# otaviog/align3d

Measured on AMD Instinct MI355X. Metric: ICP frame-pairs/sec (640x480, 3-lvl, 15 iters), higher is better.
Workload: dtype f32; 1 GPU; ms3x15 x 64 pairs/GPU, distinct frames, 640x480, 3 lvl x 15 it, HBM-resident (configs[4] shard); pairs_per_gpu=64, global_pairs=64, levels=3, distinct_frames=True, ranks_in_collective=1, collective=none

## Files before the change

align3d_amd/csrc/image_icp.hip:

```cpp
#include <cstdlib>
#include <memory>

#include "icp_engine.hpp"

using namespace a3d;

namespace {

struct LevelDesc {
  const float* src_points;
  const uint8_t* src_mask;
  const uint8_t* src_intensities;
  const float* tgt_points;
  const float* tgt_normals;
  const uint8_t* tgt_mask;
  const float* imap;
  uint32_t src_n;
  uint32_t tw, th;
  float fx, fy, cx, cy;
  uint32_t flags;
  uint32_t ppt;
  uint32_t src_w;
  const uint16_t* src_depth;
  const uint16_t* tgt_depth;
// ... 61 lines not shown
  uint32_t depth;
  float row, col;
};
struct SrcStride {
  float q, q1, r, w;
};
__device__ __forceinline__ SrcStride make_src_stride(uint32_t w) {
  w = w ? w : 1u;
  const uint32_t q = 256u / w;
  return {(float)q, (float)(q + 1u), (float)(256u - q * w), (float)w};
}
__device__ __forceinline__ void src_advance(const SrcStride& st, float row, float col, float* nrow, float* ncol) {
  const float c = col + st.r;
  const bool wrap = c >= st.w;
  *ncol = wrap ? c - st.w : c;
  *nrow = row + (wrap ? st.q1 : st.q);
}
struct BackProj {
  float fx, fy, cx, cy, scale;
  DivBy dfx, dfy;
};
struct BackProj2 {
  BackProj src, tgt;
};
__device__ __forceinline__ float uniform_f(float x) {
  return __int_as_float(__builtin_amdgcn_readfirstlane(__float_as_int(x)));
}
template <bool SHORT = false>
__device__ __forceinline__ BackProj make_backproj(const float (&k)[5], const float (&rcp_f)[2]) {
  BackProj b;
  b.fx = k[0], b.fy = k[1], b.cx = k[2], b.cy = k[3], b.scale = k[4];
  if (SHORT) {
    b.dfx = DivBy{-b.fx, rcp_f[0]}, b.dfy = DivBy{-b.fy, rcp_f[1]};
    return b;
  }
  const DivBy dx = div_prepare(b.fx), dy = div_prepare(b.fy);
  b.dfx = DivBy{uniform_f(dx.negz), uniform_f(dx.y)}, b.dfy = DivBy{uniform_f(dy.negz), uniform_f(dy.y)};
  return b;
}
constexpr int D16_TGT = 1, D16_SRC = 2;
#ifndef A3D_ICP_DEPTH16_SRC
#define A3D_ICP_DEPTH16_SRC 1
#endif
constexpr int D16_SIDES = D16_TGT | (A3D_ICP_DEPTH16_SRC ? D16_SRC : 0);
template <bool ZMASK = false, int D16 = 0>
__device__ __forceinline__ SrcPx stage_a(const LevelDesc& d, uint32_t i, bool in_range, const SrcPx* prev = nullptr,
                                         const SrcStride* stride = nullptr) {
  const uint32_t ii = in_range ? i : 0u;
  SrcPx s;
  if (D16 & D16_SRC) {
    if (prev) {
      src_advance(*stride, prev->row, prev->col, &s.row, &s.col);
    } else {
      const uint32_t r = f32_as_usize(((float)i + 0.5f) * d.src_inv_w);
      s.row = (float)r, s.col = (float)(i - __umul24(r, d.src_w));
    }
    s.depth = ld<uint16_t>(d.src_depth, ii * 2u);
    s.intensity = ld<uint8_t>(d.src_intensities, ii);
    s.live = in_range;
    return s;
  }
  s.sp = ld_v3(d.src_points, ii);
  s.intensity = ld<uint8_t>(d.src_intensities, ii);
  if (ZMASK) {
    s.live = in_range & (s.sp.z != 0.0f);
    return s;
  }
  const uint8_t mask = ld<uint8_t>(d.src_mask, ii);
  s.live = in_range & (mask != 0);
  return s;
}

struct ProjPx {
  V3 p;
  float u, v;
  V3 tp, tn;
  uint8_t tmask;
  bool live;
  _Float16 tdepth;
  uint32_t trow, tcol;
  float t00, t10, t01, t11;
};
template <bool ZMASK = false, int D16 = 0, bool CLASSIC = false, bool SHORT = false>
__device__ __forceinline__ ProjPx stage_b(const LevelDesc& d, const Pose& T, const SrcPx& s, float twf, float thf,
                                          const BackProj2& bp = BackProj2{}) {
  ProjPx o;
  V3 sp = s.sp;
  bool slive = s.live;
  if (D16 & D16_SRC) {
    sp = backproject_px_proven_f<SHORT>((float)s.depth, s.row, s.col, bp.src.cx, bp.src.cy, bp.src.scale, bp.src.dfx, bp.src.dfy);
    slive = slive & (s.depth != 0u);
  }
  o.p = transform_vector(T, sp);
  const float z = o.p.z, au = o.p.x * d.fx, av = o.p.y * d.fy;
  const DivBy dz = div_prepare(z);
  float qu = div_by(au, dz), qv = div_by(av, dz);
  if (__builtin_expect(__builtin_amdgcn_ballot_w64(!(div_den_ok(z) & div_num_ok(au) & div_num_ok(av))) != 0ull, 0))
    qu = au / z, qv = av / z;
  o.u = qu + d.cx;
  o.v = qv + d.cy;
  const float ur = o.u + 0.5f, vr = o.v + 0.5f;
  o.live = slive & !((ur <= -1.0f) | (ur >= twf) | (vr <= -1.0f) | (vr >= thf));
  const uint32_t col = (uint32_t)f32_as_i32(ur), row = (uint32_t)f32_as_i32(vr);
  const uint32_t tidx = o.live ? __umul24(row, d.tw) + col : 0u;
  if (D16 & D16_TGT) {
    o.tdepth = ld<_Float16>(d.tgt_depth, tidx * 2u);
    o.trow = row, o.tcol = col;
    o.tn = ld_v3(d.tgt_normals, tidx);
// ... 234 lines not shown
  if (st->status != A3D_OK) sa.mode = SOLVE_NONE;
  block_finish<NACC>(acc, partials + (size_t)pair * gridDim.x * GN_PARTIAL, tile, gridDim.x,
                     counters + pair, st, sa, pair);
}

__global__ void __launch_bounds__(256)
    image_icp_exact_kernel(const LevelDesc* __restrict__ descs, const JobState* __restrict__ states, Gates gt,
                           float* __restrict__ partials, int PPT) {
  float acc[GN_PARTIAL];
#pragma unroll
  for (int k = 0; k < GN_PARTIAL; ++k) acc[k] = 0.0f;
  const LevelDesc d = descs[0];
  const Pose T = states[0].pose;
  const uint32_t mw = d.tw + 2;
  const float twf = (float)d.tw, thf = (float)d.th;
  auto step_exact = [](float* a, float r, const float J[6]) {
    int t = 0;
    for (int i = 0; i < 6; ++i)
      for (int j = i; j < 6; ++j) {
        const float m = J[i] * J[j];
        a[t] = a[t] + m;
        ++t;
      }
    for (int i = 0; i < 6; ++i) {
      const float m = J[i] * r;
      a[21 + i] = a[21 + i] + m;
    }
    const float rr = r * r;
    a[27] = a[27] + rr;
    a[28] += 1.0f;
  };
  for (int k0 = 0; k0 < PPT; ++k0) {
    const uint32_t i = blockIdx.x * (256u * (uint32_t)PPT) + threadIdx.x + (uint32_t)k0 * 256u;
    const SrcPx s0 = stage_a(d, i, i < d.src_n);
    ProjPx px = stage_b(d, T, s0, twf, thf);
    const MapPx mp = stage_c(d, gt, px, mw);
    if (px.live) {
      const Terms t = stage_d<true>(d, gt, px, mp, s0.intensity, mw);
      step_exact(acc, t.rg, t.Jg);
      if (t.color) step_exact(acc + GN_ACC, t.rc, t.Jc);
    }
  }
  block_reduce_store<GN_PARTIAL, false>(acc, partials + (size_t)blockIdx.x * GN_PARTIAL);
}

#endif

template <bool ZMASK, int D16 = 0>
__device__ __forceinline__ SrcPx pixel_source_at(const LevelDesc& d, uint32_t base, int ppt, int k0,
                                                 const SrcPx* prev = nullptr, const SrcStride* stride = nullptr) {
  const uint32_t i = base + (uint32_t)k0 * 256u;
  return stage_a<ZMASK, D16>(d, i, (k0 < ppt) && (i < d.src_n), prev, stride);
}
template <bool ZMASK, int D16 = 0, bool CLASSIC = false, bool SHORT = false, bool LATE = false>
__device__ __forceinline__ void pixel_pass(const LevelDesc& d, const Gates& gt, const Pose& T, uint32_t base, int ppt,
                                           const SrcPx& s0, SrcPx sa, float (&acc)[GN_PARTIAL]) {
  const uint32_t mw = d.tw + 2;
  const float twf = (float)d.tw, thf = (float)d.th;
  BackProj2 bp{};
  if (D16 & D16_SRC) bp.src = make_backproj<SHORT>(d.src_bp, d.src_rcp_f);
  if (D16 & D16_TGT) bp.tgt = make_backproj<SHORT>(d.tgt_bp, d.tgt_rcp_f);
  SrcStride stride{};
  if (D16 & D16_SRC) stride = make_src_stride(d.src_w);
  SrcPx sb;
  ProjPx pa = stage_b<ZMASK, D16, CLASSIC, SHORT>(d, T, s0, twf, thf, bp), pb;
  uint8_t ia = s0.intensity, ib;
  auto step = [&](ProjPx& cur, uint8_t cur_i, ProjPx& nxt, uint8_t& nxt_i, const SrcPx& s_next, SrcPx& s_new, int k0) {
    Shifted sh;
    if constexpr (!CLASSIC && !LATE) sh = request_shifted(d, cur, mw);
    s_new = pixel_source_at<ZMASK, D16>(d, base, ppt, k0 + 2, &s_next, &stride);
    if constexpr (!CLASSIC) {
      __builtin_amdgcn_sched_barrier(0);
      nxt = stage_b<ZMASK, D16, false, SHORT>(d, T, s_next, twf, thf, bp);
      nxt_i = s_next.intensity;
      __builtin_amdgcn_sched_barrier(0);
      const MapPx mp = stage_c<ZMASK, D16, false, SHORT>(d, gt, cur, mw, bp, LATE ? nullptr : &sh);
      if (cur.live) {
        const Terms t = stage_d(d, gt, cur, mp, cur_i, mw, LATE ? nullptr : &sh);
        gn_step(acc, t.rg, t.Jg);
        if (t.color) gn_step(acc + GN_ACC, t.rc, t.Jc);
      }
      return;
    }
    if (D16) __builtin_amdgcn_sched_barrier(0);
    const MapPx mp = stage_c<ZMASK, D16, true, SHORT>(d, gt, cur, mw, bp);
    nxt = stage_b<ZMASK, D16, true, SHORT>(d, T, s_next, twf, thf, bp);
    nxt_i = s_next.intensity;
    if (cur.live) {
      const Terms t = stage_d(d, gt, cur, mp, cur_i, mw);
      gn_step(acc, t.rg, t.Jg);
      if (t.color) gn_step(acc + GN_ACC, t.rc, t.Jc);
    }
  };
#pragma unroll 1
  for (int k0 = 0; k0 < ppt; k0 += 2) {
    step(pa, ia, pb, ib, sa, sb, k0);
    step(pb, ib, pa, ia, sb, sa, k0 + 1);
  }
}

template <bool ZMASK, bool DEPTH16, bool CLASSIC = false, bool SHORT = false, bool LATE = false>
__global__ void __launch_bounds__(256, 1)
    image_icp_head_kernel(const LevelDesc* __restrict__ descs, const JobState* __restrict__ states_in,
                          JobState* __restrict__ states_out, Gates gt, const float* __restrict__ partials_in,
                          float* __restrict__ partials_out, uint32_t job_stride, HeadArgs head) {
  __shared__ uint32_t s_state[JOB_WORDS];
  const int pair = blockIdx.y;
  const uint32_t tile = blockIdx.x;
  float acc[GN_PARTIAL];
#pragma unroll
  for (int k = 0; k < GN_PARTIAL; ++k) acc[k] = 0.0f;
#if defined(A3D_DIAGNOSTICS) && defined(A3D_TAIL_STAMPS)
  const bool stamping = threadIdx.x == 0 && pair == 0 && tile + 1 == gridDim.x;
  unsigned long long* stamp = g_tail_stamps + 16 + 8 * ((states_out > states_in) ? 1 : 0);
#define A3D_HEAD_STAMP(k) do { if (stamping) stamp[k] = __builtin_amdgcn_s_memrealtime(); } while (0)
#else
#define A3D_HEAD_STAMP(k) do { } while (0)
#endif
  A3D_HEAD_STAMP(0);
  const LevelDesc d = descs[pair];
  const int ppt = (int)d.ppt;
  const uint32_t base = tile * (256u * (uint32_t)ppt) + threadIdx.x;
  constexpr int D16 = DEPTH16 ? D16_SIDES : 0;
  SrcStride stride{};
  if (D16 & D16_SRC) stride = make_src_stride(d.src_w);
  const SrcPx s0 = pixel_source_at<ZMASK, D16>(d, base, ppt, 0), s1 = pixel_source_at<ZMASK, D16>(d, base, ppt, 1, &s0, &stride);
  A3D_HEAD_STAMP(1);
  head_advance(states_in + pair, tile == 0 ? states_out + pair : nullptr, partials_in + (size_t)pair * job_stride, head,
               pair, s_state, tile == 0);
  A3D_HEAD_STAMP(2);
  if ((int)s_state[15] == A3D_OK) {
    auto uni = [&](int k) { return __uint_as_float(__builtin_amdgcn_readfirstlane(s_state[k])); };
    const Pose T{{uni(0), uni(1), uni(2)}, {uni(3), uni(4), uni(5), uni(6)}};
    pixel_pass<ZMASK, D16, CLASSIC, SHORT, LATE>(d, gt, T, base, ppt, s0, s1, acc);
  }
  A3D_HEAD_STAMP(3);
  block_reduce_store<GN_PARTIAL, false>(acc, partials_out + (size_t)pair * job_stride + (size_t)tile * GN_PARTIAL);
  A3D_HEAD_STAMP(4);
#undef A3D_HEAD_STAMP
}

#ifdef A3D_DIAGNOSTICS
struct PersistLevel {
  uint32_t desc_base;
  uint32_t iterations;
  uint32_t tiles;
  float weight, color_weight;
  Gates gates;
};
constexpr int PERSIST_MAX_LEVELS = 16;
constexpr uint32_t PAIR_CTRL_WORDS = 64;
constexpr uint32_t ROSTER_CLOSED = 0x80000000u;
constexpr unsigned long long ROSTER_WAIT_TICKS = 2000ull, PERSIST_SPIN_BOUND_TICKS = 200'000'000ull;
struct PersistPlan {
  uint32_t n_levels;
  uint32_t seq0;
  uint32_t counter_base;
  uint32_t finish;
  uint32_t parity;
  int trace_index0;
  int trace_stride;
  HeadArgs prev;
  PersistLevel lv[PERSIST_MAX_LEVELS];
};
struct PersistOut {
  Pose* poses;
  int32_t* status;
  float* matrices;
  unsigned long long* stamps;
};

template <bool ZMASK>
__global__ void __launch_bounds__(256, 4)
    image_icp_persistent_kernel(const LevelDesc* __restrict__ descs, uint32_t n_pairs_total, JobState* __restrict__ states,
                                float* __restrict__ partials, uint32_t partials_half, uint32_t job_stride,
                                unsigned* __restrict__ ctrl, PersistPlan plan, PersistOut out) {
  __shared__ uint32_t s_state[JOB_WORDS];
  __shared__ uint32_t s_rank, s_members;
  __shared__ int s_go;
  const int pair = blockIdx.y;
  unsigned* const counter = ctrl + (size_t)pair * PAIR_CTRL_WORDS;
  unsigned* const roster = counter + 1 + plan.parity;
  unsigned* const members = counter + 3 + plan.parity;
  float* const job_partials = partials + (size_t)pair * job_stride;
  if (threadIdx.x == 0) {
    const uint32_t old = __hip_atomic_fetch_add(roster, 1u, __ATOMIC_RELAXED, __HIP_MEMORY_SCOPE_AGENT);
    uint32_t rank = old & 0xffffu, R = 0;
// ... 345 lines not shown
    const f32x4_t t = acc0 + acc1;
    const int colx = lane & 15, row4 = (lane >> 4) * 4;
    tiles_lds[wave * 256 + (row4 + 0) * 16 + colx] = t.x;
    tiles_lds[wave * 256 + (row4 + 1) * 16 + colx] = t.y;
    tiles_lds[wave * 256 + (row4 + 2) * 16 + colx] = t.z;
    tiles_lds[wave * 256 + (row4 + 3) * 16 + colx] = t.w;
  }
  __syncthreads();
  float* job_partials = partials + (size_t)pair * gridDim.x * GN_PARTIAL;
  if (threadIdx.x < GN_PARTIAL) {
    const int e = tile_index_of_partial(threadIdx.x);
    const float v = (tiles_lds[e] + tiles_lds[256 + e]) + (tiles_lds[512 + e] + tiles_lds[768 + e]);
    __hip_atomic_store((unsigned*)(job_partials + (size_t)blockIdx.x * GN_PARTIAL) + threadIdx.x, __float_as_uint(v),
                       __ATOMIC_RELAXED, __HIP_MEMORY_SCOPE_AGENT);
  }
  SolveArgs sa = solve;
  if (st->status != A3D_OK) sa.mode = SOLVE_NONE;
  block_publish_and_finish(job_partials, gridDim.x, counters + pair, st, sa, pair);
}

#endif

__global__ void division_selftest_kernel(const float* __restrict__ num, const float* __restrict__ den, uint32_t n,
                                         unsigned* __restrict__ mismatches) {
  const uint32_t i = blockIdx.x * blockDim.x + threadIdx.x;
  if (i >= n) return;
  const float a = num[i], z = den[i];
  if (!(div_den_ok(z) && div_num_ok(a))) return;
  const float q = div_by(a, div_prepare(z)), want = a / z;
  if (__float_as_uint(q) != __float_as_uint(want)) atomicAdd(mismatches, 1u);
}

}

#ifdef A3D_DIAGNOSTICS
constexpr uint32_t CTRL_WORDS_PER_PAIR = PAIR_CTRL_WORDS;
#else
constexpr uint32_t CTRL_WORDS_PER_PAIR = 0;
#endif

struct a3d_multiscale_batch {
  a3d_context* ctx = nullptr;
  uint32_t n_pairs = 0, n_levels = 0;
  std::vector<a3d_icp_params> params;
  std::vector<Gates> gates;
  std::vector<uint32_t> tiles, ppt, group;
  std::vector<LevelDesc> h_descs;
  void* d_block = nullptr;
  LevelDesc* d_descs = nullptr;
  JobState* d_states = nullptr;
  hipEvent_t level_ready[16] = {};
  float* d_partials = nullptr;
  size_t partials_capacity = 0;
  size_t partials_half = 0;
  uint32_t max_tiles = 1;
  unsigned* d_counters = nullptr;
  uint32_t counter_base = 0;
  uint32_t persist_parity = 0;
  uint32_t persist_mask = 0;
  uint32_t persist_resident_blocks = 0;
  bool persist_disabled = false;
  bool persist_used = false;
  std::vector<uint32_t> persist_levels;
  uint32_t last_groups = 1;
  unsigned long long* d_stamps = nullptr;
  Pose* d_poses = nullptr;
  Pose* d_init = nullptr;
  int32_t* d_status = nullptr;
  double* d_readback = nullptr;
  hipEvent_t ev0 = nullptr, ev1 = nullptr;
  std::vector<hipEvent_t> kev;
  std::vector<uint8_t> kev_level;
  float last_level_ms[16] = {0};
  uint32_t last_level_launches[16] = {0};
  bool profile_kernels = false;
  uint32_t resident_blocks = 1024;
  bool zmask = false;
  bool depth16 = false;
  bool short_div = false;
  uint32_t n_streams = 1;
  hipStream_t aux_streams[3] = {nullptr, nullptr, nullptr};
  hipEvent_t ev_fork = nullptr, ev_join[3] = {nullptr, nullptr, nullptr};
  float last_total_ms = 0.f, last_kernel_ms = 0.f;
  uint64_t last_kernel_launches = 0;
  const Pose* last_init = nullptr;
  uint32_t last_levels = 0;
  float* last_matrices = nullptr;
  std::shared_ptr<UseFence> fence = std::make_shared<UseFence>();
  std::shared_ptr<UseFence> descs_uploaded = std::make_shared<UseFence>();
#ifdef A3D_DIAGNOSTICS
  unsigned* d_epochs = nullptr;
  bool use_level_kernel = false;
  uint32_t level_mask = 0;
  uint32_t level_resident_blocks = 0;
  bool use_mfma = false, merged_accumulators = false;
  bool head_solve = true;
  bool exact_solve = false;
#endif

  ~a3d_multiscale_batch() {
    fence->retire();
    hipFree(d_block);
    hipFree(d_partials);
    hipFree(d_stamps);
    if (ev0) hipEventDestroy(ev0);
    if (ev1) hipEventDestroy(ev1);
// ... 123 lines not shown
        tiling_for(d.src_n, pinned, 1, &t_own, &d.ppt);
        tiles = p == 0 ? t_own : std::max(tiles, t_own);
      }
    }
    b->tiles[l] = tiles, b->ppt[l] = ppt;
    if (((mask >> l) & 1u) && (uint64_t)tiles * P > b->persist_resident_blocks) mask &= ~(1u << l);
  }
  uint32_t run = 0;
  for (uint32_t l = L; l-- > 0;) {
    if (!((mask >> l) & 1u)) break;
    run |= 1u << l;
  }
  b->persist_mask = b->persist_disabled ? 0u : run;
}

#ifdef A3D_DIAGNOSTICS
a3d_status launch_pixel_kernel(a3d_multiscale_batch* b, uint32_t level, const SolveArgs& solve, uint32_t p0,
                               uint32_t count, hipStream_t s) {
  dim3 grid(b->tiles[level], count), block(256);
  const LevelDesc* descs = b->d_descs + (size_t)level * b->n_pairs + p0;
  JobState* states = b->d_states + p0;
  float* partials = b->d_partials + (size_t)p0 * b->max_tiles * GN_PARTIAL;
  unsigned* counters = b->d_counters + p0;
  const int ppt = (int)b->ppt[level];
  if (b->use_mfma) {
    if (b->group[level] == 2)
      hipLaunchKernelGGL((image_icp_mfma_kernel<2>), grid, block, 0, s, descs, states, b->gates[level],
                         partials, counters, solve, ppt);
    else
      hipLaunchKernelGGL((image_icp_mfma_kernel<1>), grid, block, 0, s, descs, states, b->gates[level],
                         partials, counters, solve, ppt);
  } else {
    if (b->group[level] == 4)
      hipLaunchKernelGGL((image_icp_kernel<4, false>), grid, block, 0, s, descs, states, b->gates[level], partials,
                         counters, solve, ppt);
    else if (b->group[level] == 2)
      hipLaunchKernelGGL((image_icp_kernel<2, false>), grid, block, 0, s, descs, states, b->gates[level], partials,
                         counters, solve, ppt);
    else if (b->merged_accumulators && solve.mode == SOLVE_IMAGE_ICP) {
      SolveArgs merged = solve;
      merged.mode = SOLVE_IMAGE_ICP_MERGED;
      hipLaunchKernelGGL((image_icp_kernel<1, true>), grid, block, 0, s, descs, states, b->gates[level], partials,
                         counters, merged, ppt);
    } else
      hipLaunchKernelGGL((image_icp_kernel<1, false>), grid, block, 0, s, descs, states, b->gates[level], partials,
                         counters, solve, ppt);
  }
  A3D_HIP_TRY(hipGetLastError());
  return A3D_OK;
}
#endif

a3d_status launch_head_kernel(a3d_multiscale_batch* b, uint32_t level, uint32_t seq, const HeadArgs& prev, uint32_t p0,
                              uint32_t count, hipStream_t s) {
  const uint32_t P = b->n_pairs;
  const uint32_t job_stride = b->max_tiles * GN_PARTIAL;
  const JobState* st_in = b->d_states + (size_t)(seq & 1u) * P + p0;
  JobState* st_out = b->d_states + (size_t)((seq + 1u) & 1u) * P + p0;
  const float* part_in = b->d_partials + (size_t)((seq + 1u) & 1u) * b->partials_half + (size_t)p0 * job_stride;
  float* part_out = b->d_partials + (size_t)(seq & 1u) * b->partials_half + (size_t)p0 * job_stride;
  const LevelDesc* descs = b->d_descs + (size_t)level * P + p0;
#ifdef A3D_DIAGNOSTICS
  const char* oenv = A3D_DIAG_ENV("A3D_ICP_STEP_ORDER");
  if (oenv && strcmp(oenv, "classic") == 0) {
    if (b->depth16 && level == 0)
      hipLaunchKernelGGL((image_icp_head_kernel<true, true, true>), dim3(b->tiles[level], count), dim3(256), 0, s, descs,
                         st_in, st_out, b->gates[level], part_in, part_out, job_stride, prev);
    else if (b->zmask)
      hipLaunchKernelGGL((image_icp_head_kernel<true, false, true>), dim3(b->tiles[level], count), dim3(256), 0, s, descs,
                         st_in, st_out, b->gates[level], part_in, part_out, job_stride, prev);
    else
      hipLaunchKernelGGL((image_icp_head_kernel<false, false, true>), dim3(b->tiles[level], count), dim3(256), 0, s, descs,
                         st_in, st_out, b->gates[level], part_in, part_out, job_stride, prev);
    A3D_HIP_TRY(hipGetLastError());
    return A3D_OK;
  }
  const char* renv = A3D_DIAG_ENV("A3D_ICP_RESAMPLE");
  if (renv && strcmp(renv, "late") == 0) {
    if (b->depth16 && level == 0 && b->short_div)
      hipLaunchKernelGGL((image_icp_head_kernel<true, true, false, true, true>), dim3(b->tiles[level], count), dim3(256), 0, s,
                         descs, st_in, st_out, b->gates[level], part_in, part_out, job_stride, prev);
    else if (b->depth16 && level == 0)
      hipLaunchKernelGGL((image_icp_head_kernel<true, true, false, false, true>), dim3(b->tiles[level], count), dim3(256), 0, s,
                         descs, st_in, st_out, b->gates[level], part_in, part_out, job_stride, prev);
    else if (b->zmask)
      hipLaunchKernelGGL((image_icp_head_kernel<true, false, false, false, true>), dim3(b->tiles[level], count), dim3(256), 0, s,
                         descs, st_in, st_out, b->gates[level], part_in, part_out, job_stride, prev);
    else
      hipLaunchKernelGGL((image_icp_head_kernel<false, false, false, false, true>), dim3(b->tiles[level], count), dim3(256), 0, s,
                         descs, st_in, st_out, b->gates[level], part_in, part_out, job_stride, prev);
    A3D_HIP_TRY(hipGetLastError());
    return A3D_OK;
  }
#endif
  if (b->depth16 && level == 0 && b->short_div)
    hipLaunchKernelGGL((image_icp_head_kernel<true, true, false, true>), dim3(b->tiles[level], count), dim3(256), 0, s, descs,
                       st_in, st_out, b->gates[level], part_in, part_out, job_stride, prev);
  else if (b->depth16 && level == 0)
    hipLaunchKernelGGL((image_icp_head_kernel<true, true>), dim3(b->tiles[level], count), dim3(256), 0, s, descs, st_in,
                       st_out, b->gates[level], part_in, part_out, job_stride, prev);
  else if (b->zmask)
    hipLaunchKernelGGL((image_icp_head_kernel<true, false>), dim3(b->tiles[level], count), dim3(256), 0, s, descs, st_in,
                       st_out, b->gates[level], part_in, part_out, job_stride, prev);
  else
    hipLaunchKernelGGL((image_icp_head_kernel<false, false>), dim3(b->tiles[level], count), dim3(256), 0, s, descs, st_in,
                       st_out, b->gates[level], part_in, part_out, job_stride, prev);
  A3D_HIP_TRY(hipGetLastError());
  return A3D_OK;
}

a3d_status batch_commit_descs(a3d_multiscale_batch* b) {
  const uint32_t P = b->n_pairs, L = b->n_levels;
  plan_tiling(b);
  size_t max_partials = 1;
  for (uint32_t l = 0; l < L; ++l) max_partials = std::max(max_partials, (size_t)P * b->tiles[l] * GN_PARTIAL);
  b->max_tiles = (uint32_t)(max_partials / ((size_t)P * GN_PARTIAL));
  const char* zenv = A3D_DIAG_ENV("A3D_ICP_ZMASK");
  b->zmask = !(zenv && atoi(zenv) == 0);
  for (const LevelDesc& dsc : b->h_descs) b->zmask = b->zmask && (dsc.flags & 1u);
  const char* denv = A3D_DIAG_ENV("A3D_ICP_DEPTH16");
  b->depth16 = b->zmask && L > 0 && !(denv && atoi(denv) == 0);
  for (uint32_t p = 0; p < P && b->depth16; ++p) {
    const LevelDesc& dsc = b->h_descs[p];
    b->depth16 = (dsc.flags & 2u) && dsc.src_n <= (1u << 22);
  }
  const char* senv = A3D_DIAG_ENV("A3D_ICP_SHORT_DIV");
  b->short_div = b->depth16 && !(senv && atoi(senv) == 0);
  for (uint32_t p = 0; p < P && b->short_div; ++p) b->short_div = (b->h_descs[p].flags & 4u) != 0;
  b->partials_half = max_partials;
  if (b->partials_capacity < 2 * max_partials) {
    if (b->d_partials) A3D_HIP_TRY(hipFree(b->d_partials));
    b->d_partials = nullptr;
    b->partials_capacity = 0;
    A3D_HIP_TRY(hipMalloc((void**)&b->d_partials, 2 * max_partials * sizeof(float)));
    b->partials_capacity = 2 * max_partials;
  }
  A3D_HIP_TRY(hipMemcpyAsync(b->d_descs, b->h_descs.data(), b->h_descs.size() * sizeof(LevelDesc),
                             hipMemcpyHostToDevice, b->ctx->stream));
  return A3D_OK;
}

a3d_status batch_create(a3d_context* ctx, const a3d_icp_params* params, uint32_t n_levels, uint32_t n_pairs,
                        std::unique_ptr<a3d_multiscale_batch>* out) {
  auto b = std::make_unique<a3d_multiscale_batch>();
  b->ctx = ctx;
  b->n_pairs = n_pairs;
  b->n_levels = n_levels;
  b->params.assign(params, params + n_levels);
  for (uint32_t l = 0; l < n_levels; ++l) b->gates.push_back(make_gates(params[l]));
  b->tiles.assign(n_levels, 0);
  b->ppt.assign(n_levels, 2);
  b->group.assign(n_levels, 1);
  b->h_descs.resize((size_t)n_levels * n_pairs);
  auto resident = [&](auto kernel, int fallback_per_cu) {
    int per_cu = 0;
    if (hipOccupancyMaxActiveBlocksPerMultiprocessor(&per_cu, kernel, 256, 0) != hipSuccess || per_cu < 1)
      per_cu = fallback_per_cu;
    return (uint32_t)std::max(1, ctx->num_cus) * (uint32_t)std::max(0, per_cu);
  };
  b->resident_blocks = resident(image_icp_head_kernel<true, false>, 4);
#ifdef A3D_DIAGNOSTICS
  b->persist_resident_blocks = resident(image_icp_persistent_kernel<true>, 0);
  if (const char* env = getenv("A3D_ICP_ACCUM")) {
    b->use_mfma = strcmp(env, "mfma") == 0;
    b->merged_accumulators = strcmp(env, "merged") == 0;
  }
  if (const char* env = getenv("A3D_ICP_HANDOFF")) b->head_solve = strcmp(env, "ticket") != 0;
  if (const char* env = getenv("A3D_ICP_SOLVE")) b->exact_solve = strcmp(env, "exact") == 0;
  if (const char* env = getenv("A3D_ICP_PERSISTENT")) b->use_level_kernel = atoi(env) != 0;
  if (const char* env = getenv("A3D_ICP_PERSISTENT_LEVELS")) b->level_mask = (uint32_t)strtoul(env, nullptr, 0);
  if (!b->head_solve) b->resident_blocks = resident(image_icp_kernel<1, false>, 4);
  if (b->merged_accumulators) b->resident_blocks = resident(image_icp_kernel<1, true>, 4);
  b->level_resident_blocks = resident(image_icp_level_kernel<1>, 0);
  if (b->use_level_kernel && b->level_resident_blocks) b->resident_blocks = b->level_resident_blocks;
#endif
  A3D_HIP_TRY(hipSetDevice(ctx->device));
  {
    size_t total = 0;
    auto take = [&](size_t bytes) {
      const size_t at = total;
      total += pad256(bytes);
      return at;
    };
    const size_t o_descs = take(b->h_descs.size() * sizeof(LevelDesc)), o_states = take(2 * n_pairs * sizeof(JobState)),
                 o_counters = take((size_t)n_pairs * CTRL_WORDS_PER_PAIR * sizeof(unsigned)), o_epochs = take(n_pairs * sizeof(unsigned)),
                 o_poses = take(n_pairs * sizeof(Pose)), o_init = take(n_pairs * sizeof(Pose)),
                 o_status = take(n_pairs * sizeof(int32_t)), o_readback = take(GN_PARTIAL * sizeof(double));
    A3D_HIP_TRY(hipMalloc((void**)&b->d_block, total));
    char* base = (char*)b->d_block;
// ... 112 lines not shown
    }
    plan.finish = first_per_iteration == 0 ? 1u : 0u;
    uint32_t grid_x = 1;
    for (uint32_t k = 0; k < plan.n_levels; ++k) grid_x = std::max(grid_x, plan.lv[k].tiles);
    if (b->profile_kernels && !b->d_stamps)
      A3D_HIP_TRY(hipMalloc((void**)&b->d_stamps, (size_t)P * 2 * PERSIST_MAX_LEVELS * sizeof(unsigned long long)));
    profile_level = 255;
    b->persist_levels.clear();
    for (uint32_t k = 0; k < plan.n_levels; ++k) b->persist_levels.push_back(plan.lv[k].desc_base / P);
    for (uint32_t g = 0; g < S; ++g) {
      const uint32_t p0 = (uint32_t)((uint64_t)P * g / S), p1 = (uint32_t)((uint64_t)P * (g + 1) / S);
      hipStream_t gs = g == 0 ? s : b->aux_streams[g - 1];
      PersistOut po{};
      if (plan.finish) po.poses = b->d_poses + p0, po.status = b->d_status + p0, po.matrices = d_matrices ? d_matrices + (size_t)p0 * 16 : nullptr;
      po.stamps = b->profile_kernels ? b->d_stamps + (size_t)p0 * 2 * plan.n_levels : nullptr;
      PersistPlan gp = plan;
      gp.prev.trace = d_trace;
      A3D_TRY(profile_begin(gs));
      if (b->zmask)
        hipLaunchKernelGGL(image_icp_persistent_kernel<true>, dim3(grid_x, p1 - p0), dim3(256), 0, gs, b->d_descs + p0, P,
                           b->d_states + p0, b->d_partials + (size_t)p0 * job_stride, (uint32_t)b->partials_half, job_stride,
                           b->d_counters + (size_t)p0 * PAIR_CTRL_WORDS, gp, po);
      else
        hipLaunchKernelGGL(image_icp_persistent_kernel<false>, dim3(grid_x, p1 - p0), dim3(256), 0, gs, b->d_descs + p0, P,
                           b->d_states + p0, b->d_partials + (size_t)p0 * job_stride, (uint32_t)b->partials_half, job_stride,
                           b->d_counters + (size_t)p0 * PAIR_CTRL_WORDS, gp, po);
      A3D_HIP_TRY(hipGetLastError());
      A3D_TRY(profile_end(gs));
    }
    b->persist_used = true;
    b->counter_base += published;
    for (uint32_t k = 0; k < plan.n_levels; ++k) {
      const PersistLevel& lv = plan.lv[k];
      if (!lv.iterations) continue;
      prev.weight = lv.weight, prev.color_weight = lv.color_weight, prev.mode = SOLVE_IMAGE_ICP, prev.tiles = lv.tiles;
      prev.first_in_level = lv.iterations == 1, prev.last_in_level = 1;
      seq += lv.iterations, trace_index += (int)lv.iterations;
      prev.trace_index = trace_index - 1;
    }
    finished_in_kernel = plan.finish != 0;
  }
#endif
  for (uint32_t l = first_per_iteration; l-- > 0;) {
    const a3d_icp_params& prm = b->params[l];
    profile_level = l;
    if (l < 16 && b->level_ready[l])
      for (uint32_t g = 0; g < S; ++g) A3D_HIP_TRY(hipStreamWaitEvent(g == 0 ? s : b->aux_streams[g - 1], b->level_ready[l], 0));
    if (head) {
      for (uint64_t it = 0; it < prm.max_iterations; ++it) {
        for (uint32_t g = 0; g < S; ++g) {
          const uint32_t p0 = (uint32_t)((uint64_t)P * g / S), p1 = (uint32_t)((uint64_t)P * (g + 1) / S);
          hipStream_t gs = g == 0 ? s : b->aux_streams[g - 1];
          A3D_TRY(profile_begin(gs));
          A3D_TRY(launch_head_kernel(b, l, seq, prev, p0, p1 - p0, gs));
          A3D_TRY(profile_end(gs));
        }
        prev.weight = prm.weight, prev.color_weight = prm.color_weight, prev.mode = SOLVE_IMAGE_ICP;
        prev.tiles = b->tiles[l];
        prev.first_in_level = it == 0, prev.last_in_level = it + 1 == prm.max_iterations;
        prev.trace_index = trace_index;
        ++trace_index;
        ++seq;
      }
      continue;
    }
#ifdef A3D_DIAGNOSTICS
    SolveArgs sa{};
    sa.weight = prm.weight, sa.color_weight = prm.color_weight;
    sa.mode = getenv("A3D_ICP_NOSOLVE") ? SOLVE_NONE : SOLVE_IMAGE_ICP;
    sa.trace = d_trace, sa.trace_stride = trace_stride;
    if (level_kernel || ((mask >> l) & 1u)) {
      if (prm.max_iterations == 0) continue;
      LevelPlan plan;
      plan.iterations = (uint32_t)prm.max_iterations;
      plan.epoch_base = epoch_base;
      plan.trace_base = trace_index;
      sa.first_in_level = sa.last_in_level = 0;
      sa.trace_index = 0;
      for (uint32_t g = 0; g < S; ++g) {
        const uint32_t p0 = (uint32_t)((uint64_t)P * g / S), p1 = (uint32_t)((uint64_t)P * (g + 1) / S);
        hipStream_t gs = g == 0 ? s : b->aux_streams[g - 1];
        A3D_TRY(profile_begin(gs));
        hipLaunchKernelGGL((image_icp_level_kernel<1>), dim3(b->tiles[l], p1 - p0), dim3(256), 0, gs,
                           b->d_descs + (size_t)l * P + p0, b->d_states + p0, b->gates[l],
                           b->d_partials + (size_t)p0 * b->max_tiles * GN_PARTIAL, b->d_counters + p0, b->d_epochs + p0,
                           sa, plan, (int)b->ppt[l]);
        A3D_HIP_TRY(hipGetLastError());
        A3D_TRY(profile_end(gs));
      }
      epoch_base += plan.iterations;
      trace_index += (int)plan.iterations;
      continue;
    }
    for (uint64_t it = 0; it < prm.max_iterations; ++it) {
      sa.first_in_level = it == 0, sa.last_in_level = it + 1 == prm.max_iterations;
      sa.trace_index = trace_index;
      for (uint32_t g = 0; g < S; ++g) {
        const uint32_t p0 = (uint32_t)((uint64_t)P * g / S), p1 = (uint32_t)((uint64_t)P * (g + 1) / S);
        hipStream_t gs = g == 0 ? s : b->aux_streams[g - 1];
        A3D_TRY(profile_begin(gs));
        A3D_TRY(launch_pixel_kernel(b, l, sa, p0, p1 - p0, gs));
        A3D_TRY(profile_end(gs));
      }
      ++trace_index;
    }
#endif
  }
// ... 153 lines not shown
  }
  a3d_status st = batch_enqueue(b, d_init, n_levels, nullptr, d_trace, (int)total_iters);
  if (st != A3D_OK) batch_drain_after_failure(b);
  a3d_status worst = A3D_OK;
  if (st == A3D_OK) st = read_results(b, out_pose, nullptr, &worst);
  if (st == A3D_OK && d_trace)
    if (hipMemcpy(host_trace, d_trace, total_iters * 8 * sizeof(float), hipMemcpyDeviceToHost) != hipSuccess)
      st = A3D_HIP_ERROR;
  if (d_trace) hipFree(d_trace);
  if (st != A3D_OK) return st;
  if (worst == A3D_SOLVE_FAILED) set_error("GaussNewton::solve() returned None (count == 0 or Cholesky failed)");
  return worst;
}

}

struct a3d_multiscale {
  a3d_context* ctx = nullptr;
  std::vector<a3d_icp_params> params;
  std::vector<const a3d_device_image*> targets;
};

extern "C" {

a3d_status a3d_image_icp_align(a3d_context* ctx, const a3d_icp_params* params, const a3d_device_image* target,
                               const a3d_device_image* source, const a3d_pose* init_pose, a3d_pose* out_pose) {
  A3D_REQUIRE(ctx && params && out_pose, A3D_INVALID_PARAMETER, "null argument");
  return align_single(ctx, params, 1, &target, &source, init_pose, out_pose, nullptr);
}

a3d_status a3d_image_icp_align_trace(a3d_context* ctx, const a3d_icp_params* params,
                                     const a3d_device_image* target, const a3d_device_image* source,
                                     const a3d_pose* init_pose, a3d_pose* out_pose, float* out_trace) {
  A3D_REQUIRE(ctx && params && out_pose, A3D_INVALID_PARAMETER, "null argument");
  return align_single(ctx, params, 1, &target, &source, init_pose, out_pose, out_trace);
}

static a3d_status accumulate_pass(a3d_context* ctx, const a3d_icp_params* params, const a3d_device_image* target,
                                  const a3d_device_image* source, const a3d_pose* pose, int which, double sums[GN_PARTIAL],
                                  const char* what) {
  std::unique_ptr<a3d_multiscale_batch> b;
  A3D_TRY(batch_create(ctx, params, 1, 1, &b));
  A3D_TRY(fill_desc(target, source, &b->h_descs[0]));
  A3D_TRY(batch_commit_descs(b.get()));
  Pose h_pose = pose ? pose_from_c(pose) : pose_eye();
  Pose* d_pose = b->d_init;
  a3d_status st = A3D_OK;
  hipStream_t s = ctx->stream;
  if (hipMemcpyAsync(d_pose, &h_pose, sizeof(Pose), hipMemcpyHostToDevice, s) != hipSuccess) st = A3D_HIP_ERROR;
  if (st == A3D_OK) st = launch_job_init(s, b->d_states, d_pose, 1);
  if (st == A3D_OK && which == 0) {
    HeadArgs none{};
    none.mode = SOLVE_NONE;
    st = launch_head_kernel(b.get(), 0, 0, none, 0, 1, s);
  }
#ifdef A3D_DIAGNOSTICS
  if (st == A3D_OK && which == 1) {
    hipLaunchKernelGGL(image_icp_exact_kernel, dim3(b->tiles[0]), dim3(256), 0, s, b->d_descs, b->d_states, b->gates[0],
                       b->d_partials, (int)b->ppt[0]);
    if (hipGetLastError() != hipSuccess) st = A3D_HIP_ERROR;
  }
  if (st == A3D_OK && which == 2) {
    SolveArgs sa{};
    sa.weight = params->weight, sa.color_weight = params->color_weight, sa.mode = SOLVE_NONE;
    hipLaunchKernelGGL((image_icp_kernel<1, true>), dim3(b->tiles[0], 1), dim3(256), 0, s, b->d_descs, b->d_states, b->gates[0],
                       b->d_partials, b->d_counters, sa, (int)b->ppt[0]);
    if (hipGetLastError() != hipSuccess) st = A3D_HIP_ERROR;
  }
#endif
  if (st == A3D_OK) st = launch_gn_readback(s, b->d_partials, (int)b->tiles[0], b->d_readback);
  if (st == A3D_OK && hipMemcpyAsync(sums, b->d_readback, GN_PARTIAL * sizeof(double), hipMemcpyDeviceToHost, s) != hipSuccess)
    st = A3D_HIP_ERROR;
  if (hipStreamSynchronize(s) != hipSuccess) st = A3D_HIP_ERROR;
  if (st == A3D_HIP_ERROR) set_error("%s: HIP failure: %s", what, hipGetErrorString(hipGetLastError()));
  return st;
}

a3d_status a3d_image_icp_accumulate(a3d_context* ctx, const a3d_icp_params* params, const a3d_device_image* target,
                                    const a3d_device_image* source, const a3d_pose* pose, a3d_gn_state* out_geom,
                                    a3d_gn_state* out_color) {
  A3D_REQUIRE(ctx && params, A3D_INVALID_PARAMETER, "null argument");
  double sums[GN_PARTIAL];
  A3D_TRY(accumulate_pass(ctx, params, target, source, pose, 0, sums, "a3d_image_icp_accumulate"));
  gn_states_from_sums(sums, out_geom, out_color);
  return A3D_OK;
}

#ifdef A3D_DIAGNOSTICS
a3d_status a3d_image_icp_accumulate_exact(a3d_context* ctx, const a3d_icp_params* params, const a3d_device_image* target,
                                          const a3d_device_image* source, const a3d_pose* pose, a3d_gn_state* out_geom,
                                          a3d_gn_state* out_color) {
  A3D_REQUIRE(ctx && params, A3D_INVALID_PARAMETER, "null argument");
  double sums[GN_PARTIAL];
  A3D_TRY(accumulate_pass(ctx, params, target, source, pose, 1, sums, "a3d_image_icp_accumulate_exact"));
  gn_states_from_sums(sums, out_geom, out_color);
  return A3D_OK;
}

a3d_status a3d_image_icp_accumulate_weighted(a3d_context* ctx, const a3d_icp_params* params,
                                             const a3d_device_image* target, const a3d_device_image* source,
                                             const a3d_pose* pose, a3d_gn_state* out_state) {
  A3D_REQUIRE(ctx && params && out_state, A3D_INVALID_PARAMETER, "null argument");
  double sums[GN_PARTIAL];
  A3D_TRY(accumulate_pass(ctx, params, target, source, pose, 2, sums, "a3d_image_icp_accumulate_weighted"));
  int t = 0;
  for (int i = 0; i < 6; ++i)
    for (int j = i; j < 6; ++j) {
// ... 257 lines not shown
```

Before: 26810 frame-pairs/s.

## Record per-wave live pixel steps on first iteration and skip dead steps later

On the first ICP iteration of each level the head kernel records, per wavefront, a bitmask of the pixel steps where any lane has a live source pixel (valid mask or nonzero depth). Later iterations of the same level read that mask and loop only over the live steps, skipping runs of invalid source pixels. Those later iterations recompute source coordinates directly rather than advancing incrementally, and the column computation now uses an FMA. The cost is extra mask storage packed after the partials buffer, a bitmask load and popcount per wave, and reliance on source validity staying constant across iterations within a level.

After: 26690 frame-pairs/s. About the same (-0.5%).

```diff
diff --git a/align3d_amd/csrc/image_icp.hip b/align3d_amd/csrc/image_icp.hip
--- a/align3d_amd/csrc/image_icp.hip
+++ b/align3d_amd/csrc/image_icp.hip
@@ -137,8 +137,9 @@
     if (prev) {
       src_advance(*stride, prev->row, prev->col, &s.row, &s.col);
     } else {
-      const uint32_t r = f32_as_usize(((float)i + 0.5f) * d.src_inv_w);
-      s.row = (float)r, s.col = (float)(i - __umul24(r, d.src_w));
+      const float fi = (float)i;
+      s.row = (float)f32_as_usize((fi + 0.5f) * d.src_inv_w);
+      s.col = __builtin_fmaf(-s.row, (float)d.src_w, fi);
     }
     s.depth = ld<uint16_t>(d.src_depth, ii * 2u);
     s.intensity = ld<uint8_t>(d.src_intensities, ii);
@@ -479,9 +480,42 @@
   const uint32_t i = base + (uint32_t)k0 * 256u;
   return stage_a<ZMASK, D16>(d, i, (k0 < ppt) && (i < d.src_n), prev, stride);
 }
-template <bool ZMASK, int D16 = 0, bool CLASSIC = false, bool SHORT = false, bool LATE = false>
+constexpr int LIVE_CAP = 128;
+constexpr uint32_t LIVE_WORDS_PER_BLOCK = 4 * (LIVE_CAP / 64);
+__device__ __forceinline__ uint64_t uniform_u64(uint64_t x) {
+  const uint32_t lo = __builtin_amdgcn_readfirstlane((uint32_t)x), hi = __builtin_amdgcn_readfirstlane((uint32_t)(x >> 32));
+  return ((uint64_t)hi << 32) | lo;
+}
+struct LiveSteps {
+  uint64_t w0, w1;
+  int dead;
+  __device__ __forceinline__ int count() const { return __builtin_popcountll(w0) + __builtin_popcountll(w1); }
+  __device__ __forceinline__ int pop() {
+    const bool low = w0 != 0ull;
+    const uint64_t w = low ? w0 : w1;
+    const int k = w ? (int)__builtin_ctzll(w) + (low ? 0 : 64) : dead;
+    const uint64_t rest = w & (w - 1ull);
+    w0 = low ? rest : 0ull, w1 = low ? w1 : rest;
+    return k;
+  }
+  __device__ __forceinline__ void record(int k, uint64_t lanes) {
+    uint32_t any;
+    asm("s_cmp_lg_u64 %1, 0\n\ts_cselect_b32 %0, 1, 0" : "=s"(any) : "s"(lanes) : "scc");
+    const uint64_t bit = any;
+    const uint64_t at = bit << (k & 63);
+    w0 |= k < 64 ? at : 0ull, w1 |= (k >= 64 && k < LIVE_CAP) ? at : 0ull;
+  }
+};
+template <int D16>
+__device__ __forceinline__ bool source_can_live(const SrcPx& s) {
+  return (D16 & D16_SRC) ? (s.live & (s.depth != 0u)) : s.live;
+}
+
+template <bool ZMASK, int D16 = 0, bool CLASSIC = false, bool SHORT = false, bool LATE = false, bool VISIT = true,
+          bool RECORD = false>
 __device__ __forceinline__ void pixel_pass(const LevelDesc& d, const Gates& gt, const Pose& T, uint32_t base, int ppt,
-                                           const SrcPx& s0, SrcPx sa, float (&acc)[GN_PARTIAL]) {
+                                           const SrcPx& s0, SrcPx sa, float (&acc)[GN_PARTIAL], LiveSteps* live = nullptr,
+                                           int live_count = 0) {
   const uint32_t mw = d.tw + 2;
   const float twf = (float)d.tw, thf = (float)d.th;
   BackProj2 bp{};
@@ -492,14 +526,17 @@
   SrcPx sb;
   ProjPx pa = stage_b<ZMASK, D16, CLASSIC, SHORT>(d, T, s0, twf, thf, bp), pb;
   uint8_t ia = s0.intensity, ib;
-  auto step = [&](ProjPx& cur, uint8_t cur_i, ProjPx& nxt, uint8_t& nxt_i, const SrcPx& s_next, SrcPx& s_new, int k0) {
+  if constexpr (RECORD) live->record(0, __builtin_amdgcn_ballot_w64(source_can_live<D16>(s0)));
+  auto step = [&](ProjPx& cur, uint8_t cur_i, ProjPx& nxt, uint8_t& nxt_i, const SrcPx& s_next, SrcPx& s_new, int knew) {
     Shifted sh;
     if constexpr (!CLASSIC && !LATE) sh = request_shifted(d, cur, mw);
-    s_new = pixel_source_at<ZMASK, D16>(d, base, ppt, k0 + 2, &s_next, &stride);
+    if constexpr (VISIT) s_new = pixel_source_at<ZMASK, D16>(d, base, ppt, knew, &s_next, &stride);
+    else s_new = pixel_source_at<ZMASK, D16>(d, base, ppt, knew);
     if constexpr (!CLASSIC) {
       __builtin_amdgcn_sched_barrier(0);
       nxt = stage_b<ZMASK, D16, false, SHORT>(d, T, s_next, twf, thf, bp);
       nxt_i = s_next.intensity;
+      if constexpr (RECORD) live->record(knew - 1, __builtin_amdgcn_ballot_w64(source_can_live<D16>(s_next)));
       __builtin_amdgcn_sched_barrier(0);
       const MapPx mp = stage_c<ZMASK, D16, false, SHORT>(d, gt, cur, mw, bp, LATE ? nullptr : &sh);
       if (cur.live) {
@@ -519,18 +556,28 @@
       if (t.color) gn_step(acc + GN_ACC, t.rc, t.Jc);
     }
   };
+  if constexpr (!VISIT) {
+#pragma unroll 1
+    for (int n = live_count; n > 0; n -= 2) {
+      step(pa, ia, pb, ib, sa, sb, live->pop());
+      step(pb, ib, pa, ia, sb, sa, live->pop());
+    }
+    return;
+  }
 #pragma unroll 1
   for (int k0 = 0; k0 < ppt; k0 += 2) {
-    step(pa, ia, pb, ib, sa, sb, k0);
-    step(pb, ib, pa, ia, sb, sa, k0 + 1);
-  }
-}
-
-template <bool ZMASK, bool DEPTH16, bool CLASSIC = false, bool SHORT = false, bool LATE = false>
+    step(pa, ia, pb, ib, sa, sb, k0 + 2);
+    step(pb, ib, pa, ia, sb, sa, k0 + 3);
+  }
+}
+
+constexpr int LOOP_VISIT = 0, LOOP_RECORD = 1, LOOP_SKIP = 2;
+template <bool ZMASK, bool DEPTH16, bool CLASSIC = false, bool SHORT = false, bool LATE = false,
+          int LOOP = (CLASSIC || LATE) ? LOOP_VISIT : LOOP_SKIP>
 __global__ void __launch_bounds__(256, 1)
     image_icp_head_kernel(const LevelDesc* __restrict__ descs, const JobState* __restrict__ states_in,
                           JobState* __restrict__ states_out, Gates gt, const float* __restrict__ partials_in,
-                          float* __restrict__ partials_out, uint32_t job_stride, HeadArgs head) {
+                          float* __restrict__ partials_out, uint32_t job_stride, HeadArgs head, uint64_t* live_words) {
   __shared__ uint32_t s_state[JOB_WORDS];
   const int pair = blockIdx.y;
   const uint32_t tile = blockIdx.x;
@@ -545,21 +592,48 @@
 #define A3D_HEAD_STAMP(k) do { } while (0)
 #endif
   A3D_HEAD_STAMP(0);
+  uint64_t* words = nullptr;
+  LiveSteps live{0ull, 0ull, 0};
+  if constexpr (LOOP != LOOP_VISIT) words = live_words + (((size_t)pair * gridDim.x + tile) * 4u + (threadIdx.x >> 6)) * (LIVE_CAP / 64);
   const LevelDesc d = descs[pair];
   const int ppt = (int)d.ppt;
   const uint32_t base = tile * (256u * (uint32_t)ppt) + threadIdx.x;
   constexpr int D16 = DEPTH16 ? D16_SIDES : 0;
   SrcStride stride{};
   if (D16 & D16_SRC) stride = make_src_stride(d.src_w);
-  const SrcPx s0 = pixel_source_at<ZMASK, D16>(d, base, ppt, 0), s1 = pixel_source_at<ZMASK, D16>(d, base, ppt, 1, &s0, &stride);
+  live.dead = ppt;
+  int live_count = 0;
+  SrcPx s0, s1;
+  uint64_t loaded0 = 0ull, loaded1 = 0ull;
+  if constexpr (LOOP == LOOP_SKIP) {
+    s0 = pixel_source_at<ZMASK, D16>(d, base, ppt, 0), s1 = pixel_source_at<ZMASK, D16>(d, base, ppt, 1);
+    loaded0 = words[0], loaded1 = words[1];
+  } else {
+    s0 = pixel_source_at<ZMASK, D16>(d, base, ppt, 0), s1 = pixel_source_at<ZMASK, D16>(d, base, ppt, 1, &s0, &stride);
+  }
   A3D_HEAD_STAMP(1);
   head_advance(states_in + pair, tile == 0 ? states_out + pair : nullptr, partials_in + (size_t)pair * job_stride, head,
                pair, s_state, tile == 0);
+  if constexpr (LOOP == LOOP_SKIP) {
+    live.w0 = uniform_u64(loaded0) & ~3ull, live.w1 = uniform_u64(loaded1);
+    live_count = 2 + live.count();
+  }
   A3D_HEAD_STAMP(2);
-  if ((int)s_state[15] == A3D_OK) {
+  if (__builtin_amdgcn_readfirstlane((int)s_state[15]) == A3D_OK) {
     auto uni = [&](int k) { return __uint_as_float(__builtin_amdgcn_readfirstlane(s_state[k])); };
     const Pose T{{uni(0), uni(1), uni(2)}, {uni(3), uni(4), uni(5), uni(6)}};
-    pixel_pass<ZMASK, D16, CLASSIC, SHORT, LATE>(d, gt, T, base, ppt, s0, s1, acc);
+    if constexpr (LOOP == LOOP_VISIT) {
+      pixel_pass<ZMASK, D16, CLASSIC, SHORT, LATE, true>(d, gt, T, base, ppt, s0, s1, acc);
+    } else if constexpr (LOOP == LOOP_RECORD) {
+      pixel_pass<ZMASK, D16, false, SHORT, false, true, true>(d, gt, T, base, ppt, s0, s1, acc, &live);
+    } else {
+      pixel_pass<ZMASK, D16, false, SHORT, false, false>(d, gt, T, base, ppt, s0, s1, acc, &live, live_count);
+    }
+  } else {
+    live.w0 = live.w1 = ~0ull;
+  }
+  if constexpr (LOOP == LOOP_RECORD) {
+    if ((threadIdx.x & 63u) == 0u) words[0] = live.w0, words[1] = live.w1;
   }
   A3D_HEAD_STAMP(3);
   block_reduce_store<GN_PARTIAL, false>(acc, partials_out + (size_t)pair * job_stride + (size_t)tile * GN_PARTIAL);
@@ -1011,6 +1085,9 @@
   hipEvent_t level_ready[16] = {};
   float* d_partials = nullptr;
   size_t partials_capacity = 0;
+  uint64_t* d_live = nullptr;
+  std::vector<size_t> live_offset;
+  std::vector<uint8_t> live_usable;
   size_t partials_half = 0;
   uint32_t max_tiles = 1;
   unsigned* d_counters = nullptr;
@@ -1240,7 +1317,7 @@
 #endif
 
 a3d_status launch_head_kernel(a3d_multiscale_batch* b, uint32_t level, uint32_t seq, const HeadArgs& prev, uint32_t p0,
-                              uint32_t count, hipStream_t s) {
+                              uint32_t count, hipStream_t s, bool first_in_level) {
   const uint32_t P = b->n_pairs;
   const uint32_t job_stride = b->max_tiles * GN_PARTIAL;
   const JobState* st_in = b->d_states + (size_t)(seq & 1u) * P + p0;
@@ -1248,53 +1325,46 @@
   const float* part_in = b->d_partials + (size_t)((seq + 1u) & 1u) * b->partials_half + (size_t)p0 * job_stride;
   float* part_out = b->d_partials + (size_t)(seq & 1u) * b->partials_half + (size_t)p0 * job_stride;
   const LevelDesc* descs = b->d_descs + (size_t)level * P + p0;
+  uint64_t* live_words = b->d_live + b->live_offset[level] + (size_t)p0 * b->tiles[level] * LIVE_WORDS_PER_BLOCK;
+  auto launch = [&](auto kernel) {
+    hipLaunchKernelGGL(kernel, dim3(b->tiles[level], count), dim3(256), 0, s, descs, st_in, st_out, b->gates[level], part_in,
+                       part_out, job_stride, prev, live_words);
+    A3D_HIP_TRY(hipGetLastError());
+    return A3D_OK;
+  };
+  const bool d16 = b->depth16 && level == 0;
 #ifdef A3D_DIAGNOSTICS
   const char* oenv = A3D_DIAG_ENV("A3D_ICP_STEP_ORDER");
   if (oenv && strcmp(oenv, "classic") == 0) {
-    if (b->depth16 && level == 0)
-      hipLaunchKernelGGL((image_icp_head_kernel<true, true, true>), dim3(b->tiles[level], count), dim3(256), 0, s, descs,
-                         st_in, st_out, b->gates[level], part_in, part_out, job_stride, prev);
-    else if (b->zmask)
-      hipLaunchKernelGGL((image_icp_head_kernel<true, false, true>), dim3(b->tiles[level], count), dim3(256), 0, s, descs,
-                         st_in, st_out, b->gates[level], part_in, part_out, job_stride, prev);
-    else
-      hipLaunchKernelGGL((image_icp_head_kernel<false, false, true>), dim3(b->tiles[level], count), dim3(256), 0, s, descs,
-                         st_in, st_out, b->gates[level], part_in, part_out, job_stride, prev);
-    A3D_HIP_TRY(hipGetLastError());
-    return A3D_OK;
+    if (d16) return launch(image_icp_head_kernel<true, true, true>);
+    if (b->zmask) return launch(image_icp_head_kernel<true, false, true>);
+    return launch(image_icp_head_kernel<false, false, true>);
   }
   const char* renv = A3D_DIAG_ENV("A3D_ICP_RESAMPLE");
   if (renv && strcmp(renv, "late") == 0) {
-    if (b->depth16 && level == 0 && b->short_div)
-      hipLaunchKernelGGL((image_icp_head_kernel<true, true, false, true, true>), dim3(b->tiles[level], count), dim3(256), 0, s,
-                         descs, st_in, st_out, b->gates[level], part_in, part_out, job_stride, prev);
-    else if (b->depth16 && level == 0)
-      hipLaunchKernelGGL((image_icp_head_kernel<true, true, false, false, true>), dim3(b->tiles[level], count), dim3(256), 0, s,
-                         descs, st_in, st_out, b->gates[level], part_in, part_out, job_stride, prev);
-    else if (b->zmask)
-      hipLaunchKernelGGL((image_icp_head_kernel<true, false, false, false, true>), dim3(b->tiles[level], count), dim3(256), 0, s,
-                         descs, st_in, st_out, b->gates[level], part_in, part_out, job_stride, prev);
-    else
-      hipLaunchKernelGGL((image_icp_head_kernel<false, false, false, false, true>), dim3(b->tiles[level], count), dim3(256), 0, s,
-                         descs, st_in, st_out, b->gates[level], part_in, part_out, job_stride, prev);
-    A3D_HIP_TRY(hipGetLastError());
-    return A3D_OK;
-  }
-#endif
-  if (b->depth16 && level == 0 && b->short_div)
-    hipLaunchKernelGGL((image_icp_head_kernel<true, true, false, true>), dim3(b->tiles[level], count), dim3(256), 0, s, descs,
-                       st_in, st_out, b->gates[level], part_in, part_out, job_stride, prev);
-  else if (b->depth16 && level == 0)
-    hipLaunchKernelGGL((image_icp_head_kernel<true, true>), dim3(b->tiles[level], count), dim3(256), 0, s, descs, st_in,
-                       st_out, b->gates[level], part_in, part_out, job_stride, prev);
-  else if (b->zmask)
-    hipLaunchKernelGGL((image_icp_head_kernel<true, false>), dim3(b->tiles[level], count), dim3(256), 0, s, descs, st_in,
-                       st_out, b->gates[level], part_in, part_out, job_stride, prev);
-  else
-    hipLaunchKernelGGL((image_icp_head_kernel<false, false>), dim3(b->tiles[level], count), dim3(256), 0, s, descs, st_in,
-                       st_out, b->gates[level], part_in, part_out, job_stride, prev);
-  A3D_HIP_TRY(hipGetLastError());
-  return A3D_OK;
+    if (d16 && b->short_div) return launch(image_icp_head_kernel<true, true, false, true, true>);
+    if (d16) return launch(image_icp_head_kernel<true, true, false, false, true>);
+    if (b->zmask) return launch(image_icp_head_kernel<true, false, false, false, true>);
+    return launch(image_icp_head_kernel<false, false, false, false, true>);
+  }
+  const char* venv = A3D_DIAG_ENV("A3D_ICP_DEAD_RUNS");
+  if (venv && strcmp(venv, "visit") == 0) {
+    if (d16 && b->short_div) return launch(image_icp_head_kernel<true, true, false, true, false, LOOP_VISIT>);
+    if (d16) return launch(image_icp_head_kernel<true, true, false, false, false, LOOP_VISIT>);
+    if (b->zmask) return launch(image_icp_head_kernel<true, false, false, false, false, LOOP_VISIT>);
+    return launch(image_icp_head_kernel<false, false, false, false, false, LOOP_VISIT>);
+  }
+#endif
+  if (first_in_level || !b->live_usable[level]) {
+    if (d16 && b->short_div) return launch(image_icp_head_kernel<true, true, false, true, false, LOOP_RECORD>);
+    if (d16) return launch(image_icp_head_kernel<true, true, false, false, false, LOOP_RECORD>);
+    if (b->zmask) return launch(image_icp_head_kernel<true, false, false, false, false, LOOP_RECORD>);
+    return launch(image_icp_head_kernel<false, false, false, false, false, LOOP_RECORD>);
+  }
+  if (d16 && b->short_div) return launch(image_icp_head_kernel<true, true, false, true>);
+  if (d16) return launch(image_icp_head_kernel<true, true>);
+  if (b->zmask) return launch(image_icp_head_kernel<true, false>);
+  return launch(image_icp_head_kernel<false, false>);
 }
 
 a3d_status batch_commit_descs(a3d_multiscale_batch* b) {
@@ -1316,13 +1386,24 @@
   b->short_div = b->depth16 && !(senv && atoi(senv) == 0);
   for (uint32_t p = 0; p < P && b->short_div; ++p) b->short_div = (b->h_descs[p].flags & 4u) != 0;
   b->partials_half = max_partials;
-  if (b->partials_capacity < 2 * max_partials) {
+  size_t live_words = 0;
+  b->live_offset.assign(L, 0);
+  b->live_usable.assign(L, 1);
+  for (uint32_t l = 0; l < L; ++l) {
+    b->live_offset[l] = live_words;
+    live_words += (size_t)P * b->tiles[l] * LIVE_WORDS_PER_BLOCK;
+    for (uint32_t p = 0; p < P; ++p)
+      if (b->h_descs[(size_t)l * P + p].ppt > (uint32_t)LIVE_CAP) b->live_usable[l] = 0;
+  }
+  const size_t need = 2 * max_partials + 2 * live_words;
+  if (b->partials_capacity < need) {
     if (b->d_partials) A3D_HIP_TRY(hipFree(b->d_partials));
     b->d_partials = nullptr;
     b->partials_capacity = 0;
-    A3D_HIP_TRY(hipMalloc((void**)&b->d_partials, 2 * max_partials * sizeof(float)));
-    b->partials_capacity = 2 * max_partials;
-  }
+    A3D_HIP_TRY(hipMalloc((void**)&b->d_partials, need * sizeof(float)));
+    b->partials_capacity = need;
+  }
+  b->d_live = (uint64_t*)(b->d_partials + 2 * max_partials);
   A3D_HIP_TRY(hipMemcpyAsync(b->d_descs, b->h_descs.data(), b->h_descs.size() * sizeof(LevelDesc),
                              hipMemcpyHostToDevice, b->ctx->stream));
   return A3D_OK;
@@ -1541,7 +1622,7 @@
           const uint32_t p0 = (uint32_t)((uint64_t)P * g / S), p1 = (uint32_t)((uint64_t)P * (g + 1) / S);
           hipStream_t gs = g == 0 ? s : b->aux_streams[g - 1];
           A3D_TRY(profile_begin(gs));
-          A3D_TRY(launch_head_kernel(b, l, seq, prev, p0, p1 - p0, gs));
+          A3D_TRY(launch_head_kernel(b, l, seq, prev, p0, p1 - p0, gs, it == 0));
           A3D_TRY(profile_end(gs));
         }
         prev.weight = prm.weight, prev.color_weight = prm.color_weight, prev.mode = SOLVE_IMAGE_ICP;
@@ -1801,7 +1882,7 @@
   if (st == A3D_OK && which == 0) {
     HeadArgs none{};
     none.mode = SOLVE_NONE;
-    st = launch_head_kernel(b.get(), 0, 0, none, 0, 1, s);
+    st = launch_head_kernel(b.get(), 0, 0, none, 0, 1, s, true);
   }
 #ifdef A3D_DIAGNOSTICS
   if (st == A3D_OK && which == 1) {
```
